# Tongdongq/darwin-gpu

Measured on AMD Instinct MI355X. Metric: GACT GCUPS (DP cells/s) on ~10 kb PacBio-shape reads, higher is better.
Workload: dtype int16x2 (packed); 1 GPU; ecoli10x_self_overlap; tile_size=320, tile_overlap=120, scoring=+1/-1/-1/-1, reads=4642, bases=48503677, candidates=65766, tiles=2185214, parallelism=candidates dealt round-robin over 1 GPU(s), slots_in_flight=4, passes_in_this_process=127, arch=gfx950:sramecc+:xnack-

## Files before the change

darwin-gpu_amd/csrc/gact_coop.hpp:

```cpp
#pragma once

#include "gact_lin.hpp"

namespace gact {

constexpr int kCoopBanks = 2;
constexpr int kCoopJobs = (kBlockThreads / 64) * 8 * kCoopBanks;
static_assert(kCoopJobs == 64, "a walking wave serves every job of its block, one per lane");
constexpr int kCoopCacheStride = 36;

struct CoopJob {
    uint32_t ws_off;
    int R, Q;
    int k0;
    int v0;
    int band_lim;
    uint32_t where;
    int pad_;
};
struct CoopDone { int ref_steps, query_steps, dv, redo; };

template <class L> constexpr size_t coop_bank_words() { return (size_t)L::G::kMaxFlush * L::kWalkQuads * kWsRow * 4; }
template <class L> __host__ constexpr size_t coop_ws_words(int blocks) { return (size_t)blocks * (kBlockThreads / 64) * kCoopBanks * coop_bank_words<L>(); }

// ... 117 lines not shown
    KParams kp, P16Consts kc, SeqSetDev refs, SeqSetDev qfwd, SeqSetDev qrc,
    int same_file, gact_overlap *__restrict__ out, ChainQueues cq,
    uint32_t *__restrict__ ws_all)
{
    using G = typename L::G;
    constexpr int LANES = L::kLanes;
    static_assert(LANES == kGroup && L::kWalkFmt == 3 && L::kEndAligned, "the split linear-gap layout");
    constexpr int kGroupsOfWave = 64 / LANES;
    constexpr int kGroupsPerBlock = (kBlockThreads / 64) * kGroupsOfWave;
    constexpr int kStageWords = StageGeom<L::kSlotsPerLane, LANES>::kWords;
    constexpr int kSeg = StageGeom<L::kSlotsPerLane, LANES>::kSeg;
    static_assert(((kGroupsPerBlock * kCoopBanks * kStageWords) >> 15) == 0, "stage index fits CoopJob::where");
    constexpr int kRefBytes = (G::kRefBytes + 15) & ~15;
    __shared__ __attribute__((aligned(16))) uint8_t lds[kGroupsPerBlock * kRefBytes];
    __shared__ ChainState chain_lds[kGroupsPerBlock][kCoopBanks][kSlots];
    __shared__ __attribute__((aligned(16))) uint32_t stage_lds[kGroupsPerBlock][kCoopBanks][kStageWords];
    __shared__ __attribute__((aligned(16))) CoopJob jobs[kCoopJobs];
    __shared__ CoopDone done[kCoopJobs];
    __shared__ uint32_t jstate[kCoopJobs];
    __shared__ __attribute__((aligned(16))) uint32_t cache_lds[kCoopJobs * kCoopCacheStride];
    __shared__ int bank_lds[kGroupsPerBlock][kCoopBanks][6];
    __shared__ uint32_t walk_lock;

    for (int n = threadIdx.x; n < kCoopJobs; n += kBlockThreads) jstate[n] = 0;
    if (threadIdx.x == 0) walk_lock = 0;
    __syncthreads();

    const int wave_in_block = threadIdx.x >> 6;
    WaveCtx w;
    {
        const int lane = threadIdx.x & 63;
        w.gl = lane & (LANES - 1);
        w.g = lane / LANES;
        w.slot = (blockIdx.x * (kBlockThreads / 64) + wave_in_block) * kGroupsOfWave + w.g;
        w.n_slots = gridDim.x * (kBlockThreads / 64) * kGroupsOfWave;
    }
    const int group_in_block = wave_in_block * kGroupsOfWave + w.g;
    uint8_t *ref8 = lds + group_in_block * kRefBytes;
    uint8_t *q8 = ref8;
    const uint16_t *ref16_lane = reinterpret_cast<const uint16_t *>(ref8) + (L::kRow0 - 1 - w.gl);
    uint32_t *ws_wave = ws_all + (size_t)(blockIdx.x * (kBlockThreads / 64) + wave_in_block) * (kCoopBanks * coop_bank_words<L>());
    const int job_base = (group_in_block * kSlots + (w.gl & 1)) * kCoopBanks;

    for (int b = 0; b < kCoopBanks; b++)
        if (w.gl < kSlots) { chain_lds[group_in_block][b][w.gl].phase = 2; chain_lds[group_in_block][b][w.gl].cand = -1; }
    if (w.gl == 0) {
        int *bt = &bank_lds[group_in_block][0][0];
        for (int n = 0; n < kCoopBanks * 6; n++) bt[n] = 0;
// ... 161 lines not shown
            int *bw = &bank_lds[group_in_block][bank][0];
            bw[0] = have[0] ? pt.R[0] : 0; bw[1] = pt.Q[0]; bw[2] = have[1] ? pt.R[1] : 0; bw[3] = pt.Q[1];
        }
        const bool any_here = have[0] | have[1];
        if (!__any(any_here)) {
            const bool other_busy = __builtin_amdgcn_readfirstlane(bank_lds[group_in_block][bank ^ 1][4]) != 0;
            if (!other_busy) {
                const ChainState *so = chain_lds[group_in_block][bank ^ 1];
                if (__all(exhausted && st[0].phase == 2 && st[1].phase == 2 && so[0].phase == 2 && so[1].phase == 2)) break;
                if (!second_set && !one_set) {
                    __builtin_amdgcn_s_sleep(127);
                    if (++idle_polls > 512) { second_set = true; exhausted = true; my_bucket = kBuckets; }
                }
            }
            bank ^= 1;
            continue;
        }
        const int T_end = wave_max_groups<LANES>(imax(have[0] ? Tend_h[0] : 0, have[1] ? Tend_h[1] : 0));
        const int reach0 = have[0] ? tB_h[0] + (T_end - Tend_h[0]) : 0x7fffffff;
        const int reach1 = have[1] ? tB_h[1] + (T_end - Tend_h[1]) : 0x7fffffff;
        const int tB = wave_min_groups<LANES>(imin(reach0, reach1));
        pt.col_from = imax(imin(have[0] ? pt.Q[0] : 0x7fff, have[1] ? pt.Q[1] : 0x7fff) - kp.early, 0);
        pt.band = kp.band;
        pt.shift[0] = have[0] ? T_end - Tend_h[0] : 0;
        pt.shift[1] = have[1] ? T_end - Tend_h[1] : 0;

        GACT_STAMP(t_b);
        uint32_t qb[L::kSlotsPerLane];
        uint32_t *stage = stage_lds[group_in_block][bank];
        load_pair_packed<L::kSlotsPerLane, LANES, typename L::Cols, false>(refs, qfwd, qrc, pt, w.gl, ref8, G::kRefBytes, G::kRow0, q8, G::kTileMax, qb,
                                                                          stage, typename L::Cols{});
        wave_sync();
        GACT_STAMP(t_c);

        const int wave_longest = wave_max_groups<LANES>(longest);
        const int ref_longest = ranked_longest(cq, kp, wave_longest, rank_turn, rank_cached);
        const bool rank_hi = kp.prio_bases[0] == 0 ? 16 * wave_longest > (kp.prio_bases[1] >> 8) * ref_longest
                                                   : wave_longest > kp.prio_bases[1];
        const bool rank_mid = kp.prio_bases[0] == 0 ? 16 * wave_longest > (kp.prio_bases[1] & 255) * ref_longest
                                                    : wave_longest > kp.prio_bases[0];
        if (rank_hi) __builtin_amdgcn_s_setprio(2);
        else if (rank_mid) __builtin_amdgcn_s_setprio(1);
        else __builtin_amdgcn_s_setprio(0);
        uint32_t *wsA = ws_wave + (size_t)bank * coop_bank_words<L>() + (w.g * LANES) * 4;
        uint32_t *wsB = wsA + 64 * 4;
        const uint32_t fin = L::template pass<false>(kc, w.gl, ref16_lane, qb, T_end, tB, wsA, wsB, pt);
        __builtin_amdgcn_s_setprio(3);
        const int v0A = (int)(int16_t)(__shfl(fin, L::fin_lane(pt.Q[0]), LANES) & 0xffffu);
        const int v0B = (int)(int16_t)(__shfl(fin, L::fin_lane(pt.Q[1]), LANES) >> 16);
        GACT_STAMP(t_d);
        asm volatile("s_waitcnt vmcnt(0)" ::: "memory");
        GACT_STAMP(t_e);

// ... 47 lines not shown
```

darwin-gpu_amd/csrc/gact_lin.hpp:

```cpp
#pragma once

#include "gact_p16s.hpp"

namespace gact {

#ifndef GACT_LIN_MAX3
#define GACT_LIN_MAX3 1
#endif
constexpr int kLinFloor = GACT_LIN_MAX3 ? 1024 : 0;
__host__ __device__ constexpr int lin_base(int g) { return kLinFloor + 40 * (-g) + 8; }
__device__ __forceinline__ uint32_t vconst(uint32_t s)
{
    uint32_t r;
    asm volatile("s_nop 1\n\tv_mov_b32 %0, %1" : "=v"(r) : "s"(s));
    return r;
}

__host__ inline bool p16_lin_ok(int tile, int match, int mismatch, int open, int ext)
{
    const long long steps = (long long)tile + 4 * kGroup + 64 + 48;
    return open == ext && mismatch == ext && ext <= 0 && match >= 0 &&
           p16_tagged_ok(tile, match, mismatch, open, ext) &&
           4 * ((long long)match * (tile + 2) + (long long)(-ext) * steps + kLinFloor) + 3 <= 30000 && match - ext <= 63;
}
// ... 2 lines not shown
{
    uint32_t r;
    asm("v_pk_mad_u16 %0, %1, 4, %2 op_sel_hi:[1,0,1]" : "=v"(r) : "v"(a), "v"(v_c));
    return r;
}
__device__ __forceinline__ uint32_t pk_max3f(uint32_t a, uint32_t b, uint32_t c)
{
    uint32_t r;
    asm("v_pk_maximum3_f16 %0, %1, %2, %3" : "=v"(r) : "v"(a), "v"(b), "v"(c));
    return r;
}
__device__ __forceinline__ uint32_t andn_or(uint32_t a, uint32_t b, uint32_t c)
{
    uint32_t r;
    asm("v_bitop3_b32 %0, %1, %2, %3 bitop3:0xba" : "=v"(r) : "v"(a), "v"(b), "v"(c));
    return r;
}
__device__ __forceinline__ uint32_t pk_ashr2(uint32_t a)
{
    uint32_t r;
    asm("v_pk_ashrrev_i16 %0, 2, %1 op_sel_hi:[0,1]" : "=v"(r) : "v"(a));
    return r;
}

template <int CW> struct LinWords {
    static constexpr int kWords = (CW + 1) / 2;
    static constexpr int kUint4 = (kWords + 3) / 4;
};
template <int NW, int LANES, class Fix>
__device__ __forceinline__ void lin_flush(const uint32_t (&acc)[2 * NW], uint4 *qA, uint4 *qB, Fix fix, const bool storeA, const bool storeB)
{
    constexpr int QD = (NW + 3) / 4;
    uint32_t wa[QD * 4], wb[QD * 4];
#pragma unroll
    for (int n = 0; n < QD * 4; n++) {
        wa[n] = n < NW ? fix(__builtin_amdgcn_perm(acc[n < NW ? 2 * n + 1 : 0], acc[n < NW ? 2 * n : 0], 0x05040100u)) : 0u;
        wb[n] = n < NW ? fix(__builtin_amdgcn_perm(acc[n < NW ? 2 * n + 1 : 0], acc[n < NW ? 2 * n : 0], 0x07060302u)) : 0u;
    }
    if (storeA) {
#pragma unroll
        for (int q = 0; q < QD; q++) qA[q * kWsRow] = make_uint4(wa[4 * q], wa[4 * q + 1], wa[4 * q + 2], wa[4 * q + 3]);
    }
    if (storeB) {
#pragma unroll
        for (int q = 0; q < QD; q++) qB[q * kWsRow] = make_uint4(wb[4 * q], wb[4 * q + 1], wb[4 * q + 2], wb[4 * q + 3]);
    }
}

constexpr int kLinBandDefault = 48, kLinBandMin = 24, kLinBandQuantum = 1;
struct LinBand {
    int lo[2], hi[2];
    bool full[2];
    __device__ __forceinline__ bool store(int h, int first, int last) const { return full[h] | ((last >= lo[h]) & (first <= hi[h])); }
};
__device__ __forceinline__ void lin_band_range(LinBand &b, int h, int T_end, int behind, int dj_min, int dj_max, int band, bool full)
{
    b.full[h] = full | (band <= 0);
    b.lo[h] = T_end - behind - dj_max - band;
    b.hi[h] = dj_max < 0 ? -0x40000000 : T_end - behind - imax(dj_min, 0) + band;
}

template <int C1, int C2>
__device__ __forceinline__ uint32_t dp_pass_lin_split(const P16Consts &kc, const int gl,
                                                      const uint16_t *__restrict__ ref16,
                                                      const uint32_t (&qb)[C1 + C2],
                                                      const int T_end, const int tB,
                                                      uint32_t *__restrict__ wsA, uint32_t *__restrict__ wsB,
                                                      const int band, const bool fullA, const bool fullB)
{
    constexpr int CT = C1 + C2;
    constexpr int NW = LinWords<C2>::kWords, QD = LinWords<C2>::kUint4;
    constexpr int LAG = kGroup;
    const int g = (int)(int16_t)(kc.ext & 0xffffu);
    const uint32_t gv = vconst(kc.next), g4v = vconst(kc.next4), c3v = vconst(kc.c3), onev = vconst(kc.one),
                   dtv = vconst(kc.next4 + kc.tag1),
                   c2v = vconst(kc.tag2), lut1v = vconst(0x01010101u);
    uint32_t Z1 = pk2(lin_base(g) + gl * g), Z2 = pk2(lin_base(g) + (gl + LAG) * g);
    uint32_t G[CT];
    uint32_t acc[2 * NW];
#pragma unroll
    for (int c = 0; c < CT; c++) G[c] = c < C1 ? Z1 : Z2;
#pragma unroll
    for (int c = 0; c < 2 * NW; c++) acc[c] = 0;
    uint32_t H1 = Z1, H2 = Z2;
    uint32_t Hdiag1 = Z1, Hdiag2 = Z2;

    auto lut = [&](uint32_t amount) { return kc.dsub >> (amount & 31u); };
    auto lut4 = [&](uint32_t amount) { return kc.dsub4 >> (amount & 31u); };
    uint32_t rb1 = 0, rb1b = 0, rb2 = 0, rb2b = 0;
    {
        const uint32_t w1 = ref16[1], w2 = ref16[1 - LAG];
        rb1 = lut(w1 & 0xffu); rb1b = lut(w1 >> 8); rb2 = lut(w2 & 0xffu); rb2b = lut(w2 >> 8);
    }

#define GACT_SB() __builtin_amdgcn_sched_barrier(0)
    auto upper_all = [&](uint32_t (&U)[CT], const bool tag2, const uint32_t Zr2) {
        uint32_t P[CT];
#pragma unroll
        for (int c = 0; c < CT; c++) P[c] = __builtin_amdgcn_perm(c < C1 ? rb1b : rb2b, c < C1 ? rb1 : rb2, qb[c]);
        GACT_SB();
#pragma unroll
        for (int c = 0; c < CT; c++) U[c] = (c == 0 ? Hdiag1 : c == C1 ? Hdiag2 : G[c - 1]) + P[c];
        (void)tag2;
        GACT_SB();
        if (GACT_LIN_MAX3) {
#pragma unroll
            for (int c = 0; c < CT; c++)
                U[c] = pk_max3f(U[c], c < C1 ? Z1 : Zr2, G[c]);
        } else {
#pragma unroll
            for (int c = 0; c < CT; c++) U[c] = pk_max(U[c], c < C1 ? Z1 : Zr2);
            GACT_SB();
#pragma unroll
            for (int c = 0; c < CT; c++) U[c] = pk_max(U[c], G[c]);
        }
        GACT_SB();
    };

    auto step = [&](const int t) {
        const uint32_t w1 = ref16[t + 1], w2 = ref16[t + 1 - LAG];
        Z1 += gv; Z2 += gv;
        const uint32_t Hl1 = (uint32_t)dpp_row_shr1((int)H1, (int)Z1);
        const uint32_t Hl2 = (uint32_t)dpp_row_shr1((int)H2, dpp_row_ror1((int)H1));
        uint32_t U[CT];
        upper_all(U, false, Z2);
        Hdiag1 = Hl1; Hdiag2 = Hl2;
        uint32_t Ha = Hl1, Hb = Hl2;
        static_assert(C2 >= C1, "region 2 is the longer chain");
#pragma unroll
        for (int c = 0; c < C1; c++) {
            const uint32_t Da = Ha - gv, Db = Hb - gv;
            GACT_SB();
            G[c] = pk_max(U[c], Da); G[C1 + c] = pk_max(U[C1 + c], Db);
            GACT_SB();
            Ha = G[c]; Hb = G[C1 + c];
        }
#pragma unroll
        for (int c = 2 * C1; c < CT; c++) { G[c] = pk_max(U[c], Hb - gv); Hb = G[c]; }
        H1 = Ha; H2 = Hb;
        rb1 = lut(w1 & 0xffu); rb1b = lut(w1 >> 8); rb2 = lut(w2 & 0xffu); rb2b = lut(w2 >> 8);
    };
    auto step_r1 = [&](const int t) {
        const uint32_t w1 = ref16[t + 1];
        Z1 += gv; Z2 += gv;
        const uint32_t Hl1 = (uint32_t)dpp_row_shr1((int)H1, (int)Z1);
        uint32_t P[C1], U[C1];
#pragma unroll
        for (int c = 0; c < C1; c++) P[c] = __builtin_amdgcn_perm(rb1b, rb1, qb[c]);
        GACT_SB();
#pragma unroll
        for (int c = 0; c < C1; c++) U[c] = (c == 0 ? Hdiag1 : G[c - 1]) + P[c];
        GACT_SB();
#pragma unroll
        for (int c = 0; c < C1; c++) U[c] = GACT_LIN_MAX3 ? pk_max3f(U[c], Z1, G[c]) : pk_max(pk_max(U[c], Z1), G[c]);
        GACT_SB();
        Hdiag1 = Hl1;
        uint32_t Ha = Hl1;
#pragma unroll
        for (int c = 0; c < C1; c++) { G[c] = pk_max(U[c], Ha - gv); Ha = G[c]; }
        H1 = Ha;
        rb1 = lut(w1 & 0xffu); rb1b = lut(w1 >> 8);
    };

    uint32_t Z24 = 0;
    auto step_tagged = [&](const int t) {
        const uint32_t w1 = ref16[t + 1], w2 = ref16[t + 1 - LAG];
        Z1 += gv; Z24 += g4v;
        const uint32_t Hl1 = (uint32_t)dpp_row_shr1((int)H1, (int)Z1);
        const uint32_t Hl2 = (uint32_t)dpp_row_shr1((int)H2, dpp_row_ror1((int)pk_mad4v(H1, c2v)));
        uint32_t U[CT];
        upper_all(U, true, Z24);
        Hdiag1 = Hl1; Hdiag2 = Hl2;
        uint32_t Ha = Hl1, Hb = Hl2;
        uint32_t tprev = 0;
#pragma unroll
        for (int c = 0; c < C2; c++) {
            const bool both = c < C1;
            uint32_t Da = 0;
            const uint32_t Db = Hb - dtv;
            if (both) Da = Ha - gv;
            GACT_SB();
            const uint32_t Hp = pk_max(U[C1 + c], Db);
            if (both) { G[c] = pk_max(U[c], Da); Ha = G[c]; }
            if (c > 0) acc[c - 1] = pk_shl_add4(acc[c - 1], tprev);
            GACT_SB();
            G[C1 + c] = andn_or(Hp, c3v, c2v);
            tprev = Hp & c3v;
            GACT_SB();
            Hb = G[C1 + c];
        }
        acc[C2 - 1] = pk_shl_add4(acc[C2 - 1], tprev);
        H1 = Ha; H2 = Hb;
        rb1 = lut(w1 & 0xffu); rb1b = lut(w1 >> 8); rb2 = lut4(w2 & 0xffu) + lut1v; rb2b = lut4(w2 >> 8) + lut1v;
    };
    auto step_tagged_r2 = [&](const int t) {
        const uint32_t w2 = ref16[t + 1 - LAG];
        Z24 += g4v;
        const uint32_t Hl2 = (uint32_t)dpp_row_shr1((int)H2, dpp_row_ror1((int)pk_mad4v(H1, c2v)));
        uint32_t P[C2], U[C2];
#pragma unroll
        for (int c = 0; c < C2; c++) P[c] = __builtin_amdgcn_perm(rb2b, rb2, qb[C1 + c]);
        GACT_SB();
#pragma unroll
        for (int c = 0; c < C2; c++) U[c] = (c == 0 ? Hdiag2 : G[C1 + c - 1]) + P[c];
        GACT_SB();
#pragma unroll
        for (int c = 0; c < C2; c++) U[c] = GACT_LIN_MAX3 ? pk_max3f(U[c], Z24, G[C1 + c]) : pk_max(pk_max(U[c], Z24), G[C1 + c]);
        GACT_SB();
        Hdiag2 = Hl2;
        uint32_t Hb = Hl2;
        uint32_t tprev = 0;
#pragma unroll
        for (int c = 0; c < C2; c++) {
            const uint32_t Db = Hb - dtv;
            GACT_SB();
            const uint32_t Hp = pk_max(U[c], Db);
            if (c > 0) acc[c - 1] = pk_shl_add4(acc[c - 1], tprev);
            GACT_SB();
            G[C1 + c] = andn_or(Hp, c3v, c2v);
            tprev = Hp & c3v;
            GACT_SB();
            Hb = G[C1 + c];
        }
        acc[C2 - 1] = pk_shl_add4(acc[C2 - 1], tprev);
        H2 = Hb;
        rb2 = lut4(w2 & 0xffu) + lut1v; rb2b = lut4(w2 >> 8) + lut1v;
    };
#undef GACT_SB
    auto enter_tagged = [&]() {
#pragma unroll
        for (int c = C1; c < CT; c++) G[c] = pk_mad4v(G[c], c2v);
        H2 = pk_mad4v(H2, c2v);
        Hdiag2 = pk_mad4v(Hdiag2, c2v);
        Z24 = pk_mad4v(Z2, c3v);
        rb2 = (rb2 << 2) + lut1v; rb2b = (rb2b << 2) + lut1v;
    };

    int t = 1;
    for (const int tP = imin(LAG, imin(tB - 1, T_end)); t <= tP; t++) step_r1(t);
    if (t > 1) {
#pragma unroll
        for (int c = C1; c < CT; c++) G[c] = Z2;
        H2 = Z2; Hdiag2 = Z2;
        const uint32_t w2 = ref16[t - LAG];
        rb2 = lut(w2 & 0xffu); rb2b = lut(w2 >> 8);
    }
    for (; t < tB && t <= T_end; t++) step(t);
    const bool tagged = t <= T_end;
    if (tagged) enter_tagged();
    uint4 *qA = reinterpret_cast<uint4 *>(wsA) + gl;
    uint4 *qB = reinterpret_cast<uint4 *>(wsB) + gl;
    LinBand bd;
    {
        const int q1 = (band >> 16) - 1, b = band & 0xffff;
        const int u_lo = kGroup - 1 - (gl & ~q1), u_hi = kGroup - 1 - (gl | q1);
        LinBand lo_, hi_;
        lin_band_range(lo_, 0, T_end, u_lo, C2 * u_lo, C2 * u_lo + C2 - 1, b, fullA);
        lin_band_range(hi_, 0, T_end, u_hi, C2 * u_hi, C2 * u_hi + C2 - 1, b, fullA);
        bd.lo[0] = bd.lo[1] = lo_.lo[0]; bd.hi[0] = bd.hi[1] = hi_.hi[0];
        bd.full[0] = fullA | (b <= 0); bd.full[1] = fullB | (b <= 0);
    }
    int k = 0;
    while (t + 7 <= T_end && t <= T_end - LAG) {
        for (int s8 = 0; s8 < 8; s8++, t++) step_tagged(t);
        k += 8;
        lin_flush<NW, kGroup>(acc, qA, qB, [](uint32_t w) { return w; }, bd.store(0, t - 8, t - 1), bd.store(1, t - 8, t - 1));
        qA += QD * kWsRow;
        qB += QD * kWsRow;
    }
    while (t + 7 <= T_end) {
        for (int s8 = 0; s8 < 8; s8++, t++) step_tagged_r2(t);
        k += 8;
        lin_flush<NW, kGroup>(acc, qA, qB, [](uint32_t w) { return w; }, bd.store(0, t - 8, t - 1), bd.store(1, t - 8, t - 1));
        qA += QD * kWsRow;
        qB += QD * kWsRow;
    }
    for (; t <= T_end - LAG; t++, k++) step_tagged(t);
    for (; t <= T_end; t++, k++) step_tagged_r2(t);
    if (k & 7) {
        const int sh = 2 * (8 - (k & 7));
        lin_flush<NW, kGroup>(acc, qA, qB, [sh](uint32_t w) { return ((w & 0xffffu) << sh & 0xffffu) | ((w >> 16) << sh << 16); },
                              bd.store(0, t - (k & 7), t - 1), bd.store(1, t - (k & 7), t - 1));
    }
    return tagged ? pk_ashr2(pk_sub(H2 | kc.c3, Z24)) : pk_sub(H2, Z2);
}

template <int C, int LANES, bool AMAX>
__device__ __forceinline__ uint32_t dp_pass_lin(const P16Consts &kc, const int gl,
                                                const uint16_t *__restrict__ ref16,
                                                const uint32_t (&qb)[C],
                                                const int T_end, const int tB,
                                                uint32_t *__restrict__ wsA, uint32_t *__restrict__ wsB,
                                                const int cqA, const int cqB, const int (*RQ)[2], P16Best *pb,
                                                const int col_from, const int band, const int QA, const int QB,
                                                const bool fullA, const bool fullB)
{
    constexpr int NW = LinWords<C>::kWords, QD = LinWords<C>::kUint4;
    const bool store = AMAX || gl * C + C >= col_from;
    LinBand bd;
    {
        const int q1 = AMAX ? 0 : (band >> 16) - 1, b = AMAX ? 0 : band & 0xffff;
// ... 213 lines not shown
#endif
    static constexpr int kBlocksPerCu = GACT_WIDE_LIN_BLOCKS;
    static constexpr bool kEndAligned = true;
    template <bool RAW>
    __device__ static uint32_t pass(const P16Consts &kc, int gl, const uint16_t *ref16, const uint32_t (&qb)[10], int T_end,
                                    int tB, uint32_t *wsA, uint32_t *wsB, const PairTile &pt)
    {
        static_assert(!RAW, "the linear-gap pass reads 2-bit sets");
        return dp_pass_lin<10, 32, false>(kc, gl, ref16, qb, T_end, tB, wsA, wsB, (imax(pt.Q[0], 1) - 1) % 10,
                                          (imax(pt.Q[1], 1) - 1) % 10, nullptr, nullptr, pt.col_from, pt.band, pt.Q[0], pt.Q[1],
                                          pt.full[0], pt.full[1]);
    }
    __device__ static int fin_lane(int Q) { return (imax(Q, 1) - 1) / 10; }
};

#ifndef GACT_LIN_BLOCKS_PER_CU
#define GACT_LIN_BLOCKS_PER_CU 3
#endif
template <int C1, int C2> struct SplitLayoutLin : SplitLayout<C1, C2, true> {
    static constexpr int kBlocksPerCu = GACT_LIN_BLOCKS_PER_CU;
    static constexpr int kWalkFmt = 3, kWalkQuads = LinWords<C2>::kUint4;
    static constexpr int kWalkSpan = GACT_WALK_SPAN;
    static constexpr bool kEndAligned = true;
    template <bool RAW>
    __device__ static uint32_t pass(const P16Consts &kc, int gl, const uint16_t *ref16, const uint32_t (&qb)[C1 + C2],
                                    int T_end, int tB, uint32_t *wsA, uint32_t *wsB, const PairTile &pt)
    {
        static_assert(!RAW, "the linear-gap pass reads 2-bit sets");
        return dp_pass_lin_split<C1, C2>(kc, gl, ref16, qb, T_end, tB, wsA, wsB, pt.band, pt.full[0], pt.full[1]);
    }
    __device__ static int fin_lane(int Q) { (void)Q; return kGroup - 1; }
};

template <int C1, int C2> struct SplitLayoutLinTeam : SplitLayoutLin<C1, C2> {
    static constexpr bool kTeamWalk = true;
};

}
```

darwin-gpu_amd/csrc/gact_p16.hpp:

```cpp
#pragma once

#include <type_traits>

#include "gact_chain.hpp"
#include "gact_kernels.hpp"

namespace gact {

#ifdef GACT_STAMPS
__device__ unsigned long long g_stamps[8];
__device__ unsigned long long g_stamps2[8];
__device__ unsigned long long g_timeline[4 * 4096];
__device__ unsigned long long g_wave_cycles[4096];
__device__ unsigned long long g_coop_counts[4];
#define GACT_STAMP(var) unsigned long long var = __builtin_amdgcn_s_memtime()
#define GACT_ACC(slot, t0, t1) stamp_acc[slot] += (t1) - (t0)
#else
#define GACT_STAMP(var)
#define GACT_ACC(slot, t0, t1)
#endif

#ifndef GACT_SEED_WALK_TEAM
#define GACT_SEED_WALK_TEAM 1
#endif
// ... 396 lines not shown
                const int oj = __shfl_xor(bj, mm, kGroup);
                const bool take = (ob > best) | ((ob == best) & ((oi > bi) | ((oi == bi) & (oj > bj))));
                best = take ? ob : best;
                bi = take ? oi : bi;
                bj = take ? oj : bj;
            }
            pb->best[h] = best; pb->bi[h] = bi; pb->bj[h] = bj;
        }
    }
    if (k & 7) {
        const int sh = 2 * (8 - (k & 7));
        auto just = [sh](uint32_t w) { return ((w & 0xffffu) << sh & 0xffffu) | ((w >> 16) << sh << 16); };
#pragma unroll
        for (int q = 0; q < QD; q++) {
            qA[q * kWsRow] = make_uint4(just(wordA(accO[4 * q], accF[4 * q])), just(wordA(accO[4 * q + 1], accF[4 * q + 1])),
                                        just(wordA(accO[4 * q + 2], accF[4 * q + 2])), just(wordA(accO[4 * q + 3], accF[4 * q + 3])));
            qB[q * kWsRow] = make_uint4(just(wordB(accO[4 * q], accF[4 * q])), just(wordB(accO[4 * q + 1], accF[4 * q + 1])),
                                        just(wordB(accO[4 * q + 2], accF[4 * q + 2])), just(wordB(accO[4 * q + 3], accF[4 * q + 3])));
        }
    }
}

constexpr uint32_t kLutPadRow = 31, kPermZero = 0x0c;
struct PairTile {
    int R[kSlots], Q[kSlots], shift[kSlots];
    bool reverse[kSlots];
    int64_t rp0[kSlots], qp0[kSlots];
    int comp[kSlots];
    int col_from;
    int band;
    bool full[kSlots];
};

template <int C, bool RAW, int LANES = kGroup>
__device__ __forceinline__ void load_pair(const SeqSetDev &rs, const SeqSetDev &qfwd, const SeqSetDev &qrc,
                                          const PairTile &pt, int gl, uint8_t *ref8, uint8_t *q8,
                                          uint32_t (&qb)[C])
{
    using G = GeometryP16<C, LANES>;
    GACT_STAMP(l_a);
    uint32_t *ref32 = reinterpret_cast<uint32_t *>(ref8);
    for (int k = gl; k < G::kRefBytes / 4; k += LANES) ref32[k] = RAW ? 0xffffffffu : kLutPadRow * 0x01010101u;
    wave_sync();
    GACT_STAMP(l_b);
    uint32_t rv[kSlots][C], qv[kSlots][C];
#pragma unroll
    for (int h = 0; h < kSlots; h++) {
        const SeqSetDev &qs = pt.comp[h] ? qrc : qfwd;
#pragma unroll
        for (int c = 0; c < C; c++) {
            rv[h][c] = fetch_base<RAW>(rs, slice_pos(pt.rp0[h], pt.R[h], pt.reverse[h], gl * C + c));
            qv[h][c] = fetch_base<RAW>(qs, slice_pos(pt.qp0[h], pt.Q[h], pt.reverse[h], gl * C + c));
        }
    }
#ifdef GACT_STAMPS
// ... 44 lines not shown

template <int N, int KFRONT>
__device__ __forceinline__ void cut_run(const uint32_t *seg_words, int bit0, int len, bool reverse, int d0, uint32_t (&code)[N])
{
    static_assert(N <= 32, "one 64-bit window");
    typedef __attribute__((address_space(3))) const uint32_t LdsWord;
    LdsWord *st = (LdsWord *)seg_words;
    const int lo = imax(16 * KFRONT + bit0 + (reverse ? len - d0 - N : d0), 0);
    const int wi = lo >> 4;
    const uint32_t sh = 2u * (uint32_t)(lo & 15);
    const uint32_t w0 = st[wi], w1 = st[wi + 1], w2 = st[wi + 2];
    const uint32_t x_lo = __builtin_amdgcn_alignbit(w1, w0, sh), x_hi = __builtin_amdgcn_alignbit(w2, w1, sh);
#pragma unroll
    for (int k = 0; k < N; k++) {
        const int p = reverse ? N - 1 - k : k;
        const uint32_t fwd = k < 16 ? (x_lo >> (2 * k)) & 3u : (x_hi >> (2 * (k - 16))) & 3u;
        const int pr = N - 1 - k;
        const uint32_t rev = pr < 16 ? (x_lo >> (2 * pr)) & 3u : (x_hi >> (2 * (pr - 16))) & 3u;
        (void)p;
        code[k] = reverse ? rev : fwd;
    }
}

template <int CT, int LANES, class COL, bool WRITE_Q8 = true>
__device__ __forceinline__ void load_pair_packed(const SeqSetDev &rs, const SeqSetDev &qfwd, const SeqSetDev &qrc,
                                                 const PairTile &pt, int gl, uint8_t *ref8, int ref_bytes, int row0,
                                                 uint8_t *q8, int q_stride, uint32_t (&qb)[CT], uint32_t *stage, COL)
{
    using SG = StageGeom<CT, LANES>;
    constexpr int kStageSeg = SG::kSeg;
    GACT_STAMP(l_a);
    uint32_t *ref32 = reinterpret_cast<uint32_t *>(ref8);
    for (int k = gl; k < ref_bytes / 4; k += LANES) ref32[k] = kLutPadRow * 0x01010101u;
#pragma unroll
    for (int seg = 0; seg < 4; seg++) {
        const int h = seg >> 1;
        const bool is_q = seg & 1;
        const uint32_t *words = is_q ? (pt.comp[h] ? qrc.packed : qfwd.packed) : rs.packed;
        const int64_t p0 = is_q ? pt.qp0[h] : pt.rp0[h];
        const int len = imax(is_q ? pt.Q[h] : pt.R[h], 1);
        const int64_t w0 = p0 >> 4;
        const int last = (int)(((p0 + len - 1) >> 4) - w0);
        for (int k = gl; k < kStageSeg - SG::kFront; k += LANES)
            stage[seg * kStageSeg + SG::kFront + k] = words[w0 + imin(k, last)];
    }
    wave_sync();
    GACT_STAMP(l_b);
#pragma unroll
    for (int h = 0; h < kSlots; h++) {
        const int R = pt.R[h], Q = pt.Q[h];
        const bool rev = pt.reverse[h];
        uint8_t *rrow = ref8 + (row0 + pt.shift[h]) * 2 + h;
        uint32_t rc[CT];
        cut_run<CT, SG::kFront>(stage + (2 * h) * kStageSeg, (int)(pt.rp0[h] & 15), R, rev, gl * CT, rc);
#pragma unroll
        for (int s = 0; s < CT; s++) {
            const int d = gl * CT + s;
            rrow[imin(d, R) * 2] = (uint8_t)(d < R ? 24u - rc[s] * 8u : kLutPadRow);
        }
        const uint32_t *qseg = stage + (2 * h + 1) * kStageSeg;
        const int qbit0 = (int)(pt.qp0[h] & 15);
        auto run = [&](auto first_tag, auto n_tag) {
            constexpr int S0 = decltype(first_tag)::value, N = decltype(n_tag)::value;
            const int c0 = COL::column(gl, S0, Q);
            uint32_t qc[N];
            cut_run<N, SG::kFront>(qseg, qbit0, Q, rev, c0, qc);
#pragma unroll
            for (int k = 0; k < N; k++) {
                const int dq = c0 + k;
                const bool real = (unsigned)dq < (unsigned)Q;
                if (WRITE_Q8 && real) q8[h * q_stride + dq] = (uint8_t)(24u - qc[k] * 8u);
                const uint32_t keep = h ? 0xff00ffffu : 0xffffff00u;
                const uint32_t mine = (h ? qb[S0 + k] : kPermZero * 0x01010101u);
                qb[S0 + k] = real ? (mine & keep) | ((qc[k] + 4u * h) << (16 * h)) : mine;
            }
        };
        COL::for_each_run(run);
    }
#ifdef GACT_STAMPS
    asm volatile("s_waitcnt lgkmcnt(0)" ::: "memory");
    GACT_STAMP(l_c);
// ... 70 lines not shown
    constexpr int LANES = L::kLanes;
    constexpr int kGroupsOfWave = 64 / LANES;
    constexpr int kGroupsPerBlock = (kBlockThreads / 64) * kGroupsOfWave;
    __shared__ __attribute__((aligned(16))) uint8_t lds[kGroupsPerBlock * G::kGroupLds];
    __shared__ ChainState chain_lds[kGroupsPerBlock][kSlots];
    constexpr bool kTeamWalk = walk_by_team<L>();
    constexpr int kStageHalf = (StageGeom<L::kSlotsPerLane, LANES>::kWords / kSlots + 3) & ~3;
    constexpr int kScratchWords = walk_scratch_words<L, kTeamWalk>() > kStageHalf ? walk_scratch_words<L, kTeamWalk>() : kStageHalf;
    __shared__ __attribute__((aligned(16))) uint32_t tb_lds[kGroupsPerBlock][kSlots][kScratchWords];

    WaveCtx w;
    {
        const int lane = threadIdx.x & 63;
        const int wave = (blockIdx.x * blockDim.x + threadIdx.x) >> 6;
        w.gl = lane & (LANES - 1);
        w.g = lane / LANES;
        w.slot = wave * kGroupsOfWave + w.g;
        w.n_slots = ((gridDim.x * blockDim.x) >> 6) * kGroupsOfWave;
    }
    const int group_in_block = (threadIdx.x >> 6) * kGroupsOfWave + w.g;
    uint8_t *ref8 = lds + group_in_block * G::kGroupLds;
    uint8_t *q8 = ref8 + G::kRefBytes;
    const uint16_t *ref16_lane = reinterpret_cast<const uint16_t *>(ref8) + (L::kRow0 - 1 - w.gl);
    constexpr int kWsPerTile = LANES / kGroup;
    static_assert(G::kWsWords <= kWsPerTile * Geometry<20>::kWsWords || L::kSlotsPerLane > 20, "workspace stride");
    uint32_t *wsA = ws_all + (size_t)(w.slot / kGroupsOfWave) * (8 * (size_t)kp.ws_words) + (w.g * LANES) * 4;
    uint32_t *wsB = wsA + 64 * 4;

    ChainState *st = chain_lds[group_in_block];
    if (w.gl < kSlots) { st[w.gl].phase = 2; st[w.gl].cand = -1; }
    wave_sync();
    bool exhausted = false;
    int my_bucket = 0;
    int bucket_first = 0;
    if (cq.leave_longest > 0) {
        int acc = 0;
        while (bucket_first < kBuckets && (acc += cq.bucket_count[bucket_first]) <= cq.leave_longest) bucket_first++;
        if (bucket_first >= kBuckets) bucket_first = 0;
    }
    bool second_set = false;
    constexpr bool one_set = !TWO_SETS;
    int idle_polls = 0;
    int rank_turn = 0, rank_cached = 0;
    __builtin_amdgcn_s_setprio(3);
#ifdef GACT_STAMPS
    unsigned long long stamp_acc[8] = {0, 0, 0, 0, 0, 0, 0, 0};
// ... 59 lines not shown
            pt.full[h] = s.full != 0;
            if (pk.have) longest = imax(longest, chain_remaining(s));
            Tend_h[h] = L::last_step(pk.R, pk.Q);
            tB_h[h] = L::first_pointer_step(pk.R, pk.Q, kp.early);
            wave_sync();
            if (w.gl == 0) st[h] = s;
            wave_sync();
        }
        const bool any_here = have[0] | have[1];
        if (!__any(any_here)) {
            if (__all(exhausted && st[0].phase == 2 && st[1].phase == 2)) break;
            if (!second_set && !one_set) {
                __builtin_amdgcn_s_sleep(127);
                if (++idle_polls > 512) { second_set = true; exhausted = true; my_bucket = kBuckets; }
            }
            continue;
        }
        const int T_end = wave_max_groups<LANES>(imax(have[0] ? Tend_h[0] : 0, have[1] ? Tend_h[1] : 0));
        const int reach0 = have[0] ? tB_h[0] + (T_end - Tend_h[0]) : 0x7fffffff;
        const int reach1 = have[1] ? tB_h[1] + (T_end - Tend_h[1]) : 0x7fffffff;
        const int tB = wave_min_groups<LANES>(imin(reach0, reach1));
        pt.col_from = imax(imin(have[0] ? pt.Q[0] : 0x7fff, have[1] ? pt.Q[1] : 0x7fff) - kp.early, 0);
        pt.band = kp.band;
        pt.shift[0] = have[0] ? (L::kEndAligned ? T_end - Tend_h[0] : imax(0, tB - tB_h[0])) : 0;
        pt.shift[1] = have[1] ? (L::kEndAligned ? T_end - Tend_h[1] : imax(0, tB - tB_h[1])) : 0;

        GACT_STAMP(t_b);
        uint32_t qb[L::kSlotsPerLane];
        L::template load<RAW>(refs, qfwd, qrc, pt, w.gl, ref8, q8, qb, tb_lds[group_in_block][0]);
        wave_sync();
        GACT_STAMP(t_c);

        const int wave_longest = wave_max_groups<LANES>(longest);
        const int ref_longest = ranked_longest(cq, kp, wave_longest, rank_turn, rank_cached);
        const bool rank_hi = kp.prio_bases[0] == 0 ? 16 * wave_longest > (kp.prio_bases[1] >> 8) * ref_longest
                                                   : wave_longest > kp.prio_bases[1];
        const bool rank_mid = kp.prio_bases[0] == 0 ? 16 * wave_longest > (kp.prio_bases[1] & 255) * ref_longest
                                                    : wave_longest > kp.prio_bases[0];
        if (rank_hi) __builtin_amdgcn_s_setprio(2);
        else if (rank_mid) __builtin_amdgcn_s_setprio(1);
        else __builtin_amdgcn_s_setprio(0);
        const uint32_t fin = L::template pass<RAW>(kc, w.gl, ref16_lane, qb, T_end, tB, wsA, wsB, pt);
        __builtin_amdgcn_s_setprio(3);
        int v0_h[kSlots] = {0, 0};
        if (L::kWalkFmt == 3 || L::kWalkFmt == 4) {
            v0_h[0] = (int)(int16_t)(__shfl(fin, L::fin_lane(pt.Q[0]), LANES) & 0xffffu);
// ... 237 lines not shown
```

darwin-gpu_amd/csrc/gact_p16s.hpp:

```cpp
#pragma once

#include "gact_p16.hpp"

namespace gact {

template <int C1, int C2> struct GeometrySplit {
    static constexpr int CT = C1 + C2;
    static constexpr int kTileMax = CT * kGroup;
    static constexpr int W1 = C1 * kGroup, W2 = C2 * kGroup;
    static constexpr int kLag = kGroup;
    static constexpr int kMaxSteps = kTileMax + kGroup + kLag;
    static constexpr int kQuads = (C2 + 3) / 4;
    static constexpr int kRow0 = kGroup + kLag;
    static constexpr int kRefEntries = kRow0 + kMaxSteps + kGroup + 8;
    static constexpr int kRefBytes = kRefEntries * 2;
    static constexpr int kQueryBytes = kTileMax * kSlots;
    static constexpr int kGroupLds = (kRefBytes + kQueryBytes + 15) & ~15;
    static constexpr int kMaxFlush = (kMaxSteps + 7) / 8 + 1;
    static constexpr int kWsWords = kMaxFlush * kQuads * 4 * kGroup;
};

__device__ __forceinline__ int dpp_row_ror1(int v)
{
    return __builtin_amdgcn_mov_dpp(v, 0x121, 0xF, 0xF, false);
}

template <int C2> __device__ __forceinline__ int split_last_step(int R, int Q)
{
    return (R > 0 && Q > 0) ? R + (kGroup - 1) + kGroup : 0;
}

template <int C2> __device__ __forceinline__ int split_first_pointer_step(int R, int Q, int early)
{
    const int r_first = imax(1, R - early + 1);
    const int j_first = imax(1, Q - early + 1);
    const int jj = j_first + (C2 * kGroup - Q);
    return r_first + (jj - 1) / C2 + kGroup;
// ... 300 lines not shown
```

darwin-gpu_amd/csrc/gact_roles.hpp:

```cpp
#pragma once

#include "gact_lin.hpp"

namespace gact {

#ifndef GACT_ROLE_DP_WAVES
#define GACT_ROLE_DP_WAVES 10
#endif
constexpr int kRoleDp = GACT_ROLE_DP_WAVES;
constexpr int kRoleWalk = kRoleDp > 7 ? 2 : 1;
constexpr int kRoleThreads = 64 * (kRoleDp + kRoleWalk);
constexpr int kRoleBanks = 2;
constexpr int kRoleJobs = kRoleDp * 8;
constexpr int kRoleJobsPerWalker = kRoleJobs / kRoleWalk;
static_assert(kRoleDp % kRoleWalk == 0 && kRoleJobsPerWalker <= 64, "a walker wave serves whole DP waves, a lane per tile slot");
constexpr int kRoleCacheStride = 36;

struct WalkJob {
    uint32_t seq;
    uint32_t ws_off;
    int R, Q;
    int k0;
    int v0;
    int band_lim;
// ... 146 lines not shown
{
    using G = typename L::G;
    constexpr int LANES = L::kLanes;
    static_assert(LANES == kGroup && L::kWalkFmt == 3 && L::kEndAligned, "the split linear-gap layout");
    constexpr int kGroupsOfWave = 64 / LANES;
    constexpr int kDpGroups = kRoleDp * kGroupsOfWave;
    constexpr int kStageWords = StageGeom<L::kSlotsPerLane, LANES>::kWords;
    constexpr int kSeg = StageGeom<L::kSlotsPerLane, LANES>::kSeg;
    static_assert(((kDpGroups * kRoleBanks * kStageWords) >> 15) == 0, "stage index fits WalkJob::where");
    __shared__ __attribute__((aligned(16))) uint8_t lds[kDpGroups * G::kGroupLds];
    __shared__ ChainState chain_lds[kDpGroups][kRoleBanks][kSlots];
    __shared__ __attribute__((aligned(16))) uint32_t stage_lds[kDpGroups][kRoleBanks][kStageWords];
    __shared__ WalkJob jobs[kRoleJobs][kRoleBanks];
    __shared__ WalkDone done[kRoleJobs][kRoleBanks];
    __shared__ __attribute__((aligned(16))) uint32_t cache_lds[kRoleJobs * kRoleCacheStride];
    __shared__ int dp_finished;
    __shared__ int bank_lds[kDpGroups][kRoleBanks][6];

    for (int n = threadIdx.x; n < kRoleJobs * kRoleBanks; n += kRoleThreads) {
        (&jobs[0][0])[n].seq = 0;
        (&done[0][0])[n].seq = 0;
    }
    if (threadIdx.x == 0) dp_finished = 0;
    __syncthreads();

    const int wave_in_block = threadIdx.x >> 6;
    if (wave_in_block >= kRoleDp) {
        __builtin_amdgcn_s_setprio(3);
        role_walker<L>(kp, ws_all, jobs, done, &stage_lds[0][0][0], cache_lds, &dp_finished);
        return;
    }

    WaveCtx w;
    {
        const int lane = threadIdx.x & 63;
        w.gl = lane & (LANES - 1);
        w.g = lane / LANES;
        w.slot = (blockIdx.x * kRoleDp + wave_in_block) * kGroupsOfWave + w.g;
        w.n_slots = gridDim.x * kRoleDp * kGroupsOfWave;
    }
    const int group_in_block = wave_in_block * kGroupsOfWave + w.g;
    uint8_t *ref8 = lds + group_in_block * G::kGroupLds;
    uint8_t *q8 = ref8 + G::kRefBytes;
    const uint16_t *ref16_lane = reinterpret_cast<const uint16_t *>(ref8) + (L::kRow0 - 1 - w.gl);
    uint32_t *ws_wave = ws_all + (size_t)(blockIdx.x * kRoleDp + wave_in_block) * (kRoleBanks * role_bank_words<L>());
    const int job_lane = wave_in_block * 8 + w.g * kSlots + (w.gl & 1);
// ... 144 lines not shown
            int *bw = &bank_lds[group_in_block][bank][0];
            bw[0] = have[0] ? pt.R[0] : 0; bw[1] = pt.Q[0]; bw[2] = have[1] ? pt.R[1] : 0; bw[3] = pt.Q[1];
        }
        const bool any_here = have[0] | have[1];
        if (!__any(any_here)) {
            const bool other_busy = __builtin_amdgcn_readfirstlane(bank_lds[group_in_block][bank ^ 1][4]) != 0;
            if (!other_busy) {
                const ChainState *so = chain_lds[group_in_block][bank ^ 1];
                if (__all(exhausted && st[0].phase == 2 && st[1].phase == 2 && so[0].phase == 2 && so[1].phase == 2)) break;
                if (!second_set && !one_set) {
                    __builtin_amdgcn_s_sleep(127);
                    if (++idle_polls > 512) { second_set = true; exhausted = true; my_bucket = kBuckets; }
                }
            }
            bank ^= 1;
            continue;
        }
        const int T_end = wave_max_groups<LANES>(imax(have[0] ? Tend_h[0] : 0, have[1] ? Tend_h[1] : 0));
        const int reach0 = have[0] ? tB_h[0] + (T_end - Tend_h[0]) : 0x7fffffff;
        const int reach1 = have[1] ? tB_h[1] + (T_end - Tend_h[1]) : 0x7fffffff;
        const int tB = wave_min_groups<LANES>(imin(reach0, reach1));
        pt.col_from = imax(imin(have[0] ? pt.Q[0] : 0x7fff, have[1] ? pt.Q[1] : 0x7fff) - kp.early, 0);
        pt.band = kp.band;
        pt.shift[0] = have[0] ? T_end - Tend_h[0] : 0;
        pt.shift[1] = have[1] ? T_end - Tend_h[1] : 0;

        GACT_STAMP(t_b);
        uint32_t qb[L::kSlotsPerLane];
        uint32_t *stage = stage_lds[group_in_block][bank];
        L::template load<false>(refs, qfwd, qrc, pt, w.gl, ref8, q8, qb, stage);
        wave_sync();
        GACT_STAMP(t_c);

        const int wave_longest = wave_max_groups<LANES>(longest);
        const int ref_longest = ranked_longest(cq, kp, wave_longest, rank_turn, rank_cached);
        const bool rank_hi = kp.prio_bases[0] == 0 ? 16 * wave_longest > (kp.prio_bases[1] >> 8) * ref_longest
                                                   : wave_longest > kp.prio_bases[1];
        const bool rank_mid = kp.prio_bases[0] == 0 ? 16 * wave_longest > (kp.prio_bases[1] & 255) * ref_longest
                                                    : wave_longest > kp.prio_bases[0];
        if (rank_hi) __builtin_amdgcn_s_setprio(2);
        else if (rank_mid) __builtin_amdgcn_s_setprio(1);
        else __builtin_amdgcn_s_setprio(0);
        uint32_t *wsA = ws_wave + (size_t)bank * role_bank_words<L>() + (w.g * LANES) * 4;
        uint32_t *wsB = wsA + 64 * 4;
        const uint32_t fin = L::template pass<false>(kc, w.gl, ref16_lane, qb, T_end, tB, wsA, wsB, pt);
        __builtin_amdgcn_s_setprio(3);
// ... 54 lines not shown
```

Before: 8618 GCUPS.

## Replace register shift LUT with LDS table lookup and prefetched ref bytes in linear pass

The linear-gap DP inner step used to compute substitution rows by shifting a packed constant by each reference byte. It now looks them up in a small LDS table holding plain and tagged rows, with padding rows set to zero. Reference bytes are fetched one step early through a pointer, and the row lookup is placed between scheduled instruction groups so LDS latency can be hidden. It also unrolls the step loops by two and eight, and shrinks the ref padding. The cost is extra LDS reads on the critical step and a table fill plus barrier at kernel start.

Result: faster. 8961 GCUPS (median of 6 runs) (+4.0%).

```diff
diff --git a/darwin-gpu_amd/csrc/gact_coop.hpp b/darwin-gpu_amd/csrc/gact_coop.hpp
--- a/darwin-gpu_amd/csrc/gact_coop.hpp
+++ b/darwin-gpu_amd/csrc/gact_coop.hpp
@@ -163,8 +163,10 @@
     __shared__ int bank_lds[kGroupsPerBlock][kCoopBanks][6];
     __shared__ uint32_t walk_lock;
 
+    uint32_t *const lin_lut = LinLutLds<L::kLutWords>::get();
     for (int n = threadIdx.x; n < kCoopJobs; n += kBlockThreads) jstate[n] = 0;
     if (threadIdx.x == 0) walk_lock = 0;
+    lin_lut_fill(lin_lut, kc, (int)threadIdx.x);
     __syncthreads();
 
     const int wave_in_block = threadIdx.x >> 6;
@@ -372,13 +374,14 @@
         const int tB = wave_min_groups<LANES>(imin(reach0, reach1));
         pt.col_from = imax(imin(have[0] ? pt.Q[0] : 0x7fff, have[1] ? pt.Q[1] : 0x7fff) - kp.early, 0);
         pt.band = kp.band;
+        pt.lut = lin_lut;
         pt.shift[0] = have[0] ? T_end - Tend_h[0] : 0;
         pt.shift[1] = have[1] ? T_end - Tend_h[1] : 0;
 
         GACT_STAMP(t_b);
         uint32_t qb[L::kSlotsPerLane];
         uint32_t *stage = stage_lds[group_in_block][bank];
-        load_pair_packed<L::kSlotsPerLane, LANES, typename L::Cols, false>(refs, qfwd, qrc, pt, w.gl, ref8, G::kRefBytes, G::kRow0, q8, G::kTileMax, qb,
+        load_pair_packed<L::kSlotsPerLane, LANES, typename L::Cols, false, kLinPadRow>(refs, qfwd, qrc, pt, w.gl, ref8, G::kRefBytes, G::kRow0, q8, G::kTileMax, qb,
                                                                           stage, typename L::Cols{});
         wave_sync();
         GACT_STAMP(t_c);
diff --git a/darwin-gpu_amd/csrc/gact_lin.hpp b/darwin-gpu_amd/csrc/gact_lin.hpp
--- a/darwin-gpu_amd/csrc/gact_lin.hpp
+++ b/darwin-gpu_amd/csrc/gact_lin.hpp
@@ -48,6 +48,7 @@
     asm("v_pk_ashrrev_i16 %0, 2, %1 op_sel_hi:[0,1]" : "=v"(r) : "v"(a));
     return r;
 }
+
 
 template <int CW> struct LinWords {
     static constexpr int kWords = (CW + 1) / 2;
@@ -92,7 +93,8 @@
                                                       const uint32_t (&qb)[C1 + C2],
                                                       const int T_end, const int tB,
                                                       uint32_t *__restrict__ wsA, uint32_t *__restrict__ wsB,
-                                                      const int band, const bool fullA, const bool fullB)
+                                                      const int band, const bool fullA, const bool fullB,
+                                                      const uint32_t *lut_lds)
 {
     constexpr int CT = C1 + C2;
     constexpr int NW = LinWords<C2>::kWords, QD = LinWords<C2>::kUint4;
@@ -100,7 +102,7 @@
     const int g = (int)(int16_t)(kc.ext & 0xffffu);
     const uint32_t gv = vconst(kc.next), g4v = vconst(kc.next4), c3v = vconst(kc.c3), onev = vconst(kc.one),
                    dtv = vconst(kc.next4 + kc.tag1),
-                   c2v = vconst(kc.tag2), lut1v = vconst(0x01010101u);
+                   c2v = vconst(kc.tag2);
     uint32_t Z1 = pk2(lin_base(g) + gl * g), Z2 = pk2(lin_base(g) + (gl + LAG) * g);
     uint32_t G[CT];
     uint32_t acc[2 * NW];
@@ -111,15 +113,26 @@
     uint32_t H1 = Z1, H2 = Z2;
     uint32_t Hdiag1 = Z1, Hdiag2 = Z2;
 
-    auto lut = [&](uint32_t amount) { return kc.dsub >> (amount & 31u); };
-    auto lut4 = [&](uint32_t amount) { return kc.dsub4 >> (amount & 31u); };
-    uint32_t rb1 = 0, rb1b = 0, rb2 = 0, rb2b = 0;
-    {
-        const uint32_t w1 = ref16[1], w2 = ref16[1 - LAG];
-        rb1 = lut(w1 & 0xffu); rb1b = lut(w1 >> 8); rb2 = lut(w2 & 0xffu); rb2b = lut(w2 >> 8);
-    }
+    typedef __attribute__((address_space(3))) const uint8_t LdsByte;
+    typedef __attribute__((address_space(3))) const uint32_t LdsWord;
+    LdsByte *const lut_plain = (LdsByte *)lut_lds, *const lut_tagged = (LdsByte *)(lut_lds + 1);
+    auto row = [](LdsByte *table, uint32_t stream_byte) { return *(LdsWord *)(table + stream_byte); };
+    LdsByte *rp = (LdsByte *)(ref16 + (1 - LAG));
+    uint32_t rb1 = row(lut_plain, rp[2 * LAG]), rb1b = row(lut_plain, rp[2 * LAG + 1]);
+    uint32_t rb2 = row(lut_plain, rp[0]), rb2b = row(lut_plain, rp[1]);
+    rp += 2;
 
 #define GACT_SB() __builtin_amdgcn_sched_barrier(0)
+    uint32_t sb1 = 0, sb1b = 0, sb2 = 0, sb2b = 0;
+    auto ask_bytes = [&](const bool r1, const bool r2) {
+        if (r2) { sb2 = rp[0]; sb2b = rp[1]; }
+        if (r1) { sb1 = rp[2 * LAG]; sb1b = rp[2 * LAG + 1]; }
+        rp += 2;
+    };
+    auto ask_rows = [&](const bool r1, const bool r2, const bool tag2) {
+        if (r1) { rb1 = row(lut_plain, sb1); rb1b = row(lut_plain, sb1b); }
+        if (r2) { rb2 = row(tag2 ? lut_tagged : lut_plain, sb2); rb2b = row(tag2 ? lut_tagged : lut_plain, sb2b); }
+    };
     auto upper_all = [&](uint32_t (&U)[CT], const bool tag2, const uint32_t Zr2) {
         uint32_t P[CT];
 #pragma unroll
@@ -127,7 +140,7 @@
         GACT_SB();
 #pragma unroll
         for (int c = 0; c < CT; c++) U[c] = (c == 0 ? Hdiag1 : c == C1 ? Hdiag2 : G[c - 1]) + P[c];
-        (void)tag2;
+        ask_rows(true, true, tag2);
         GACT_SB();
         if (GACT_LIN_MAX3) {
 #pragma unroll
@@ -143,8 +156,8 @@
         GACT_SB();
     };
 
-    auto step = [&](const int t) {
-        const uint32_t w1 = ref16[t + 1], w2 = ref16[t + 1 - LAG];
+    auto step = [&]() {
+        ask_bytes(true, true);
         Z1 += gv; Z2 += gv;
         const uint32_t Hl1 = (uint32_t)dpp_row_shr1((int)H1, (int)Z1);
         const uint32_t Hl2 = (uint32_t)dpp_row_shr1((int)H2, dpp_row_ror1((int)H1));
@@ -164,10 +177,9 @@
 #pragma unroll
         for (int c = 2 * C1; c < CT; c++) { G[c] = pk_max(U[c], Hb - gv); Hb = G[c]; }
         H1 = Ha; H2 = Hb;
-        rb1 = lut(w1 & 0xffu); rb1b = lut(w1 >> 8); rb2 = lut(w2 & 0xffu); rb2b = lut(w2 >> 8);
-    };
-    auto step_r1 = [&](const int t) {
-        const uint32_t w1 = ref16[t + 1];
+    };
+    auto step_r1 = [&]() {
+        ask_bytes(true, false);
         Z1 += gv; Z2 += gv;
         const uint32_t Hl1 = (uint32_t)dpp_row_shr1((int)H1, (int)Z1);
         uint32_t P[C1], U[C1];
@@ -176,6 +188,7 @@
         GACT_SB();
 #pragma unroll
         for (int c = 0; c < C1; c++) U[c] = (c == 0 ? Hdiag1 : G[c - 1]) + P[c];
+        ask_rows(true, false, false);
         GACT_SB();
 #pragma unroll
         for (int c = 0; c < C1; c++) U[c] = GACT_LIN_MAX3 ? pk_max3f(U[c], Z1, G[c]) : pk_max(pk_max(U[c], Z1), G[c]);
@@ -185,12 +198,11 @@
 #pragma unroll
         for (int c = 0; c < C1; c++) { G[c] = pk_max(U[c], Ha - gv); Ha = G[c]; }
         H1 = Ha;
-        rb1 = lut(w1 & 0xffu); rb1b = lut(w1 >> 8);
     };
 
     uint32_t Z24 = 0;
-    auto step_tagged = [&](const int t) {
-        const uint32_t w1 = ref16[t + 1], w2 = ref16[t + 1 - LAG];
+    auto step_tagged = [&]() {
+        ask_bytes(true, true);
         Z1 += gv; Z24 += g4v;
         const uint32_t Hl1 = (uint32_t)dpp_row_shr1((int)H1, (int)Z1);
         const uint32_t Hl2 = (uint32_t)dpp_row_shr1((int)H2, dpp_row_ror1((int)pk_mad4v(H1, c2v)));
@@ -217,10 +229,9 @@
         }
         acc[C2 - 1] = pk_shl_add4(acc[C2 - 1], tprev);
         H1 = Ha; H2 = Hb;
-        rb1 = lut(w1 & 0xffu); rb1b = lut(w1 >> 8); rb2 = lut4(w2 & 0xffu) + lut1v; rb2b = lut4(w2 >> 8) + lut1v;
-    };
-    auto step_tagged_r2 = [&](const int t) {
-        const uint32_t w2 = ref16[t + 1 - LAG];
+    };
+    auto step_tagged_r2 = [&]() {
+        ask_bytes(false, true);
         Z24 += g4v;
         const uint32_t Hl2 = (uint32_t)dpp_row_shr1((int)H2, dpp_row_ror1((int)pk_mad4v(H1, c2v)));
         uint32_t P[C2], U[C2];
@@ -229,6 +240,7 @@
         GACT_SB();
 #pragma unroll
         for (int c = 0; c < C2; c++) U[c] = (c == 0 ? Hdiag2 : G[C1 + c - 1]) + P[c];
+        ask_rows(false, true, true);
         GACT_SB();
 #pragma unroll
         for (int c = 0; c < C2; c++) U[c] = GACT_LIN_MAX3 ? pk_max3f(U[c], Z24, G[C1 + c]) : pk_max(pk_max(U[c], Z24), G[C1 + c]);
@@ -250,7 +262,6 @@
         }
         acc[C2 - 1] = pk_shl_add4(acc[C2 - 1], tprev);
         H2 = Hb;
-        rb2 = lut4(w2 & 0xffu) + lut1v; rb2b = lut4(w2 >> 8) + lut1v;
     };
 #undef GACT_SB
     auto enter_tagged = [&]() {
@@ -259,19 +270,20 @@
         H2 = pk_mad4v(H2, c2v);
         Hdiag2 = pk_mad4v(Hdiag2, c2v);
         Z24 = pk_mad4v(Z2, c3v);
-        rb2 = (rb2 << 2) + lut1v; rb2b = (rb2b << 2) + lut1v;
+        rb2 = row(lut_tagged, rp[-2]); rb2b = row(lut_tagged, rp[-1]);
     };
 
     int t = 1;
-    for (const int tP = imin(LAG, imin(tB - 1, T_end)); t <= tP; t++) step_r1(t);
+    for (const int tP = imin(LAG, imin(tB - 1, T_end)); t <= tP; t++) step_r1();
     if (t > 1) {
 #pragma unroll
         for (int c = C1; c < CT; c++) G[c] = Z2;
         H2 = Z2; Hdiag2 = Z2;
-        const uint32_t w2 = ref16[t - LAG];
-        rb2 = lut(w2 & 0xffu); rb2b = lut(w2 >> 8);
-    }
-    for (; t < tB && t <= T_end; t++) step(t);
+        rb2 = row(lut_plain, rp[-2]); rb2b = row(lut_plain, rp[-1]);
+    }
+    const int tU = imin(tB - 1, T_end);
+    for (; t + 1 <= tU; t += 2) { step(); step(); }
+    if (t <= tU) { step(); t++; }
     const bool tagged = t <= T_end;
     if (tagged) enter_tagged();
     uint4 *qA = reinterpret_cast<uint4 *>(wsA) + gl;
@@ -288,21 +300,23 @@
     }
     int k = 0;
     while (t + 7 <= T_end && t <= T_end - LAG) {
-        for (int s8 = 0; s8 < 8; s8++, t++) step_tagged(t);
+#pragma unroll
+        for (int s8 = 0; s8 < 8; s8++, t++) step_tagged();
         k += 8;
         lin_flush<NW, kGroup>(acc, qA, qB, [](uint32_t w) { return w; }, bd.store(0, t - 8, t - 1), bd.store(1, t - 8, t - 1));
         qA += QD * kWsRow;
         qB += QD * kWsRow;
     }
     while (t + 7 <= T_end) {
-        for (int s8 = 0; s8 < 8; s8++, t++) step_tagged_r2(t);
+#pragma unroll
+        for (int s8 = 0; s8 < 8; s8++, t++) step_tagged_r2();
         k += 8;
         lin_flush<NW, kGroup>(acc, qA, qB, [](uint32_t w) { return w; }, bd.store(0, t - 8, t - 1), bd.store(1, t - 8, t - 1));
         qA += QD * kWsRow;
         qB += QD * kWsRow;
     }
-    for (; t <= T_end - LAG; t++, k++) step_tagged(t);
-    for (; t <= T_end; t++, k++) step_tagged_r2(t);
+    for (; t <= T_end - LAG; t++, k++) step_tagged();
+    for (; t <= T_end; t++, k++) step_tagged_r2();
     if (k & 7) {
         const int sh = 2 * (8 - (k & 7));
         lin_flush<NW, kGroup>(acc, qA, qB, [sh](uint32_t w) { return ((w & 0xffffu) << sh & 0xffffu) | ((w >> 16) << sh << 16); },
@@ -562,12 +576,22 @@
     static constexpr int kWalkFmt = 3, kWalkQuads = LinWords<C2>::kUint4;
     static constexpr int kWalkSpan = GACT_WALK_SPAN;
     static constexpr bool kEndAligned = true;
+    static constexpr int kLutWords = kLinLutWords;
+    using Base = SplitLayout<C1, C2, true>;
+    template <bool RAW>
+    __device__ static void load(const SeqSetDev &rs, const SeqSetDev &qf, const SeqSetDev &qr,
+                                const PairTile &pt, int gl, uint8_t *ref8, uint8_t *q8, uint32_t (&qb)[C1 + C2], uint32_t *stage)
+    {
+        static_assert(!RAW, "the linear-gap pass reads 2-bit sets");
+        load_pair_packed<C1 + C2, kGroup, typename Base::Cols, true, kLinPadRow>(rs, qf, qr, pt, gl, ref8, Base::G::kRefBytes, Base::G::kRow0, q8,
+                                                                                 Base::G::kTileMax, qb, stage, typename Base::Cols{});
+    }
     template <bool RAW>
     __device__ static uint32_t pass(const P16Consts &kc, int gl, const uint16_t *ref16, const uint32_t (&qb)[C1 + C2],
                                     int T_end, int tB, uint32_t *wsA, uint32_t *wsB, const PairTile &pt)
     {
         static_assert(!RAW, "the linear-gap pass reads 2-bit sets");
-        return dp_pass_lin_split<C1, C2>(kc, gl, ref16, qb, T_end, tB, wsA, wsB, pt.band, pt.full[0], pt.full[1]);
+        return dp_pass_lin_split<C1, C2>(kc, gl, ref16, qb, T_end, tB, wsA, wsB, pt.band, pt.full[0], pt.full[1], pt.lut);
     }
     __device__ static int fin_lane(int Q) { (void)Q; return kGroup - 1; }
 };
diff --git a/darwin-gpu_amd/csrc/gact_p16.hpp b/darwin-gpu_amd/csrc/gact_p16.hpp
--- a/darwin-gpu_amd/csrc/gact_p16.hpp
+++ b/darwin-gpu_amd/csrc/gact_p16.hpp
@@ -442,6 +442,8 @@
 }
 
 constexpr uint32_t kLutPadRow = 31, kPermZero = 0x0c;
+constexpr uint32_t kLinPadRow = 32;
+constexpr int kLinLutWords = 10;
 struct PairTile {
     int R[kSlots], Q[kSlots], shift[kSlots];
     bool reverse[kSlots];
@@ -450,7 +452,23 @@
     int col_from;
     int band;
     bool full[kSlots];
+    const uint32_t *lut;
 };
+
+__device__ __forceinline__ void lin_lut_fill(uint32_t *lut, const P16Consts &kc, const int tid)
+{
+    if (tid < kLinLutWords) {
+        const uint32_t b = 8u * ((uint32_t)tid >> 1), base = (tid & 1) ? kc.dsub4 : kc.dsub;
+        lut[tid] = (b < kLinPadRow ? base >> b : 0u) + ((tid & 1) ? 0x01010101u : 0u);
+    }
+}
+template <int N> struct LinLutLds {
+    __device__ __forceinline__ static uint32_t *get() { __shared__ __attribute__((aligned(8))) uint32_t words[N]; return words; }
+};
+template <> struct LinLutLds<0> { __device__ __forceinline__ static uint32_t *get() { return nullptr; } };
+
+template <class L, class = void> struct lin_lut_words { static constexpr int value = 0; };
+template <class L> struct lin_lut_words<L, std::void_t<decltype(L::kLutWords)>> { static constexpr int value = L::kLutWords; };
 
 template <int C, bool RAW, int LANES = kGroup>
 __device__ __forceinline__ void load_pair(const SeqSetDev &rs, const SeqSetDev &qfwd, const SeqSetDev &qrc,
@@ -541,7 +559,7 @@
     }
 }
 
-template <int CT, int LANES, class COL, bool WRITE_Q8 = true>
+template <int CT, int LANES, class COL, bool WRITE_Q8 = true, uint32_t PAD_ROW = kLutPadRow>
 __device__ __forceinline__ void load_pair_packed(const SeqSetDev &rs, const SeqSetDev &qfwd, const SeqSetDev &qrc,
                                                  const PairTile &pt, int gl, uint8_t *ref8, int ref_bytes, int row0,
                                                  uint8_t *q8, int q_stride, uint32_t (&qb)[CT], uint32_t *stage, COL)
@@ -550,7 +568,7 @@
     constexpr int kStageSeg = SG::kSeg;
     GACT_STAMP(l_a);
     uint32_t *ref32 = reinterpret_cast<uint32_t *>(ref8);
-    for (int k = gl; k < ref_bytes / 4; k += LANES) ref32[k] = kLutPadRow * 0x01010101u;
+    for (int k = gl; k < ref_bytes / 4; k += LANES) ref32[k] = PAD_ROW * 0x01010101u;
 #pragma unroll
     for (int seg = 0; seg < 4; seg++) {
         const int h = seg >> 1;
@@ -575,7 +593,7 @@
 #pragma unroll
         for (int s = 0; s < CT; s++) {
             const int d = gl * CT + s;
-            rrow[imin(d, R) * 2] = (uint8_t)(d < R ? 24u - rc[s] * 8u : kLutPadRow);
+            rrow[imin(d, R) * 2] = (uint8_t)(d < R ? 24u - rc[s] * 8u : PAD_ROW);
         }
         const uint32_t *qseg = stage + (2 * h + 1) * kStageSeg;
         const int qbit0 = (int)(pt.qp0[h] & 15);
@@ -692,6 +710,11 @@
     uint8_t *ref8 = lds + group_in_block * G::kGroupLds;
     uint8_t *q8 = ref8 + G::kRefBytes;
     const uint16_t *ref16_lane = reinterpret_cast<const uint16_t *>(ref8) + (L::kRow0 - 1 - w.gl);
+    uint32_t *const lin_lut = LinLutLds<lin_lut_words<L>::value>::get();
+    if constexpr (lin_lut_words<L>::value > 0) {
+        lin_lut_fill(lin_lut, kc, (int)threadIdx.x);
+        __syncthreads();
+    }
     constexpr int kWsPerTile = LANES / kGroup;
     static_assert(G::kWsWords <= kWsPerTile * Geometry<20>::kWsWords || L::kSlotsPerLane > 20, "workspace stride");
     uint32_t *wsA = ws_all + (size_t)(w.slot / kGroupsOfWave) * (8 * (size_t)kp.ws_words) + (w.g * LANES) * 4;
@@ -797,6 +820,7 @@
         const int tB = wave_min_groups<LANES>(imin(reach0, reach1));
         pt.col_from = imax(imin(have[0] ? pt.Q[0] : 0x7fff, have[1] ? pt.Q[1] : 0x7fff) - kp.early, 0);
         pt.band = kp.band;
+        pt.lut = lin_lut;
         pt.shift[0] = have[0] ? (L::kEndAligned ? T_end - Tend_h[0] : imax(0, tB - tB_h[0])) : 0;
         pt.shift[1] = have[1] ? (L::kEndAligned ? T_end - Tend_h[1] : imax(0, tB - tB_h[1])) : 0;
 
diff --git a/darwin-gpu_amd/csrc/gact_p16s.hpp b/darwin-gpu_amd/csrc/gact_p16s.hpp
--- a/darwin-gpu_amd/csrc/gact_p16s.hpp
+++ b/darwin-gpu_amd/csrc/gact_p16s.hpp
@@ -12,7 +12,7 @@
     static constexpr int kMaxSteps = kTileMax + kGroup + kLag;
     static constexpr int kQuads = (C2 + 3) / 4;
     static constexpr int kRow0 = kGroup + kLag;
-    static constexpr int kRefEntries = kRow0 + kMaxSteps + kGroup + 8;
+    static constexpr int kRefEntries = kRow0 + kMaxSteps + kGroup;
     static constexpr int kRefBytes = kRefEntries * 2;
     static constexpr int kQueryBytes = kTileMax * kSlots;
     static constexpr int kGroupLds = (kRefBytes + kQueryBytes + 15) & ~15;
diff --git a/darwin-gpu_amd/csrc/gact_roles.hpp b/darwin-gpu_amd/csrc/gact_roles.hpp
--- a/darwin-gpu_amd/csrc/gact_roles.hpp
+++ b/darwin-gpu_amd/csrc/gact_roles.hpp
@@ -192,6 +192,8 @@
         (&done[0][0])[n].seq = 0;
     }
     if (threadIdx.x == 0) dp_finished = 0;
+    uint32_t *const lin_lut = LinLutLds<L::kLutWords>::get();
+    lin_lut_fill(lin_lut, kc, (int)threadIdx.x);
     __syncthreads();
 
     const int wave_in_block = threadIdx.x >> 6;
@@ -382,6 +384,7 @@
         const int tB = wave_min_groups<LANES>(imin(reach0, reach1));
         pt.col_from = imax(imin(have[0] ? pt.Q[0] : 0x7fff, have[1] ? pt.Q[1] : 0x7fff) - kp.early, 0);
         pt.band = kp.band;
+        pt.lut = lin_lut;
         pt.shift[0] = have[0] ? T_end - Tend_h[0] : 0;
         pt.shift[1] = have[1] ? T_end - Tend_h[1] : 0;
 
```
